# ArtoriasAbyssslayer/HashModNFFBanks-IDR

Hardware: AMD Instinct MI355X
Metric: rays/sec fwd+bwd (hash+SDF MLP) (higher is better)
Workload: dtype f32; 1 GPU; DTU-shaped synthetic uniform-sphere rays, MultiResHash L=16 T=2^19 F=2 (BASELINE.json configs[1]), full IDR training step (forward + IDRLoss + backward + clip + Adam), weights held at the geometric initialisation (lr = 0): the SURVEY.md 8(d) workload; grid_config=C2, rays_per_gpu=2048, global_rays=2048, parallelism=single GPU, world=1, ranks_seen=1, step=HIP-graph captured static-shape step

## Files before the change

hashmodnffbanks_idr_amd/csrc/hm_trace.hip:

```cpp
#include "hm_common.h"

#include <stdlib.h>
#include <string.h>

extern "C" int hm_trace_march_tail(const hm_grid_desc *desc, const hm_mlp_desc *mlp, const float *table,
                                   const float *B_fourier, int frac_mode, int body16, const void *trace_args, int first,
                                   int rounds, void *stream);

extern "C" int hm_trace_secant_persistent(const hm_grid_desc *desc, const hm_mlp_desc *mlp, const float *table,
                                          const float *B_fourier, int frac_mode, int tile_points, const void *trace_args,
                                          int n_iters, int scan_rule, void *stream);

extern "C" int hm_trace_scan_secant(const hm_grid_desc *desc, const hm_mlp_desc *mlp, const float *table,
                                    const float *B_fourier, int frac_mode, const void *trace_args, int n_iters,
                                    int64_t scan_off, int64_t scan_capacity, int c_prev1, int grid1, int c_prev2,
                                    int grid2, void *stream);

extern "C" int hm_sdf_fwd_fill(const hm_grid_desc *desc, const hm_mlp_desc *mlp, const float *x, int64_t n,
                               const float *table, const float *B_fourier, float *out, int frac_mode, const int32_t *n_dev,
                               const float *x_fill, float *out_fill, const int32_t *n_fill_dev, const int32_t *prev_dev,
                               int prev_grid, int *grid64_out, void *stream);

namespace {

constexpr int kTB = 256;

#include "hm_trace_dev.h"

__global__ __launch_bounds__(kTB) void trace_init_kernel(TraceArgs a) {
    const int64_t i = (int64_t)blockIdx.x * kTB + threadIdx.x;
    if (i >= a.n) return;
    trace_init_ray(a, i, a.w.cnt + C_ROUND0, 0);
}

__global__ __launch_bounds__(kTB) void trace_advance_kernel(TraceArgs a, int round) {
    const int64_t i = (int64_t)blockIdx.x * kTB + threadIdx.x;
    if (i >= a.n) return;
    trace_advance_ray(a, i, a.w.cnt + C_ROUND0 + round, 0);
}

__global__ __launch_bounds__(kTB) void trace_finalize_kernel(TraceArgs a) {
    const int64_t i = (int64_t)blockIdx.x * kTB + threadIdx.x;
    if (i >= a.n) return;
    const TraceWs &w = a.w;
    if (w.stage[i] != ST_DONE) atomicAdd(w.cnt + C_UNFINISHED, 1);
    const float t_s = w.t_s[i], t_e = w.t_e[i];
    a.out_mask[i] = t_s < t_e;
    a.out_t[i] = t_s;
    float px = 0.0f, py = 0.0f, pz = 0.0f;
    if (a.hit[i] || w.cnt[C_ANY_LIVE]) along(a, i, t_s, px, py, pz);
    a.out_pts[i * 3] = px; a.out_pts[i * 3 + 1] = py; a.out_pts[i * 3 + 2] = pz;
    const bool samp = w.live_s[i] != 0;
    w.is_samp[i] = samp;
    if (samp) w.list_samp[atomicAdd(w.cnt + C_NSAMP, 1)] = (int32_t)i;
}

__global__ __launch_bounds__(kTB) void ray_samples_kernel(TraceArgs a, const int32_t *list, int c_n, int c_npts,
                                                          const float *lo_arr, const float *hi_arr,
                                                          const float *fr, int c_base, int per_ray) {
    const int64_t gid = (int64_t)blockIdx.x * kTB + threadIdx.x;
    const TraceWs &w = a.w;
    const int32_t n_list = w.cnt[c_n];
    const int64_t base = c_base == -2 ? a.sel_off : (c_base >= 0 ? w.cnt[c_base] : 0);
    if (gid == 0) {
        w.cnt[c_npts] = n_list * per_ray;
        if (c_base != -2) w.cnt[C_BIG_PTS] = (int32_t)base + n_list * per_ray;
    }
    const int64_t m = gid / per_ray;
    if (m >= n_list) return;
    int s = (int)(gid - m * per_ray);
    if (per_ray < a.n_steps && s == per_ray - 1) s = a.n_steps - 1;
    const int64_t i = list[m];
    const float lo = lo_arr[i], hi = hi_arr[i];
    const float t = __fadd_rn(lo, __fmul_rn(fr[s], __fsub_rn(hi, lo)));
    float px, py, pz;
    along(a, i, t, px, py, pz);
    const int64_t o = base + gid;
    w.pts[o * 3] = px; w.pts[o * 3 + 1] = py; w.pts[o * 3 + 2] = pz;
}

__global__ __launch_bounds__(kTB) void sampler_head_kernel(TraceArgs a) {
    const int64_t m = (int64_t)blockIdx.x * kTB + threadIdx.x;
    const TraceWs &w = a.w;
    if (m >= w.cnt[C_NSAMP]) return;
    const int64_t i = w.list_samp[m];
    const float *v = w.vals + m * (a.head + 1);
    bool neg = false;
    for (int s = 0; s < a.head; ++s) neg = neg || (v[s] < 0.0f);
    const bool resolved = neg && a.obj[i] != 0;
    w.tail_slot[m] = resolved ? -1 : atomicAdd(w.cnt + C_NSAMP2, 1);
}

__global__ __launch_bounds__(kTB) void sampler_tail_points_kernel(TraceArgs a) {
    const int64_t gid = (int64_t)blockIdx.x * kTB + threadIdx.x;
    const TraceWs &w = a.w;
    const int per = a.n_steps - a.head - 1;
    if (gid == 0) {
        w.cnt[C_TAIL_PTS] = w.cnt[C_NSAMP2] * per;
        w.cnt[C_NSAMP_PTS] = w.cnt[C_HEAD_PTS] + w.cnt[C_NSAMP2] * per;
    }
    const int64_t m = gid / per;
    if (m >= w.cnt[C_NSAMP]) return;
    const int32_t q = w.tail_slot[m];
    if (q < 0) return;
    const int j = (int)(gid - m * per);
    const int64_t i = w.list_samp[m];
    const float lo = w.t_s[i], hi = w.t_e[i];
    const float t = __fadd_rn(lo, __fmul_rn(a.fracs[a.head + j], __fsub_rn(hi, lo)));
    float px, py, pz;
    along(a, i, t, px, py, pz);
    const int64_t o = a.tail_off + (int64_t)q * per + j;
    w.pts[o * 3] = px; w.pts[o * 3 + 1] = py; w.pts[o * 3 + 2] = pz;
}

__global__ __launch_bounds__(kTB) void sampler_reduce_kernel(TraceArgs a) {
    const int64_t m = (int64_t)blockIdx.x * kTB + threadIdx.x;
    const TraceWs &w = a.w;
    if (m >= w.cnt[C_NSAMP]) return;
    const int64_t i = w.list_samp[m];
    const int n = a.n_steps;
    const bool lazy = a.head > 0;
    const int32_t tq = lazy ? w.tail_slot[m] : 0;
    const float *v_head = lazy ? w.vals + m * (a.head + 1) : w.vals + m * n;
    const float *v_tail = lazy ? w.vals + a.tail_off + (int64_t)(tq < 0 ? 0 : tq) * (n - a.head - 1) - a.head : v_head;
    const int head = a.head;
    auto v = [&](int s) -> float {
        if (!lazy) return v_head[s];
        if (s < head) return v_head[s];
        return s == n - 1 ? v_head[head] : v_tail[s];
    };
    const int n_scan = (lazy && tq < 0) ? head : n;
    int first = 0, amin = 0, bad = 0;
    float best_tmp = 0.0f, best_v = 0.0f;
    auto visit = [&](int s, float x) {
        bad += !isfinite(x);
        const float sg = (x > 0.0f) ? 1.0f : ((x < 0.0f) ? -1.0f : 0.0f);
        const float tmp = sg * (float)(n - s);
        if (s == 0 || tmp < best_tmp) { best_tmp = tmp; first = s; }
        if (s == 0 || x < best_v) { best_v = x; amin = s; }
    };
    if (!lazy && (n & 3) == 0 && (reinterpret_cast<uintptr_t>(v_head) & 15u) == 0) {
        const float4 *row = reinterpret_cast<const float4 *>(v_head);
#pragma unroll 5
        for (int g4 = 0; g4 < n / 4; ++g4) {
            const float4 x4 = row[g4];
            visit(4 * g4, x4.x); visit(4 * g4 + 1, x4.y); visit(4 * g4 + 2, x4.z); visit(4 * g4 + 3, x4.w);
        }
    } else {
        for (int s = 0; s < n_scan; ++s) visit(s, v(s));
    }
    const float lo = w.t_s[i], hi = w.t_e[i];
    auto t_at = [&](int s) { return __fadd_rn(lo, __fmul_rn(a.fracs[s], __fsub_rn(hi, lo))); };
    const float v_first = v(first);
    const bool net_hit = v_first < 0.0f;
    const bool true_obj = a.obj[i] != 0;
    const int pick = (true_obj && net_hit) ? first : amin;
    float t_out = t_at(pick);
    float px, py, pz;
    along(a, i, t_out, px, py, pz);
    a.out_mask[i] = net_hit;
    const bool sec = a.training ? (net_hit && true_obj) : net_hit;
    if (sec) {
        const int lo_idx = first > 0 ? first - 1 : n - 1;
        const float z_hi = t_at(first), v_hi = v_first, z_lo = t_at(lo_idx), v_lo = v(lo_idx);
        if (lazy && tq < 0 && lo_idx == n - 1 && !isfinite(v_lo)) ++bad;
        const float z = secant_z(v_lo, v_hi, z_lo, z_hi);
        const int32_t q = atomicAdd(w.cnt + C_NSEC, 1);
        w.list_sec[q] = (int32_t)i;
        w.z_lo[q] = z_lo; w.z_hi[q] = z_hi; w.v_lo[q] = v_lo; w.v_hi[q] = v_hi; w.z[q] = z;
        if (a.n_secant == 0) {
            t_out = z;
            along(a, i, z, px, py, pz);
        }
    }
    if (bad) atomicAdd(w.cnt + C_NONFINITE, bad);
    a.out_t[i] = t_out;
    w.t_s[i] = t_out;
    a.out_pts[i * 3] = px; a.out_pts[i * 3 + 1] = py; a.out_pts[i * 3 + 2] = pz;
}

__global__ __launch_bounds__(kTB) void secant_points_kernel(TraceArgs a) {
    const int64_t q = (int64_t)blockIdx.x * kTB + threadIdx.x;
    const TraceWs &w = a.w;
    if (q >= w.cnt[C_NSEC]) return;
    float px, py, pz;
    along(a, w.list_sec[q], w.z[q], px, py, pz);
    w.pts[q * 3] = px; w.pts[q * 3 + 1] = py; w.pts[q * 3 + 2] = pz;
}

__global__ __launch_bounds__(kTB) void secant_advance_kernel(TraceArgs a, int last) {
    const int64_t q = (int64_t)blockIdx.x * kTB + threadIdx.x;
    if (q >= a.w.cnt[C_NSEC]) return;
    secant_advance_ray(a, q, last);
}

__global__ __launch_bounds__(kTB) void tail_prepare_kernel(TraceArgs a) {
    const int64_t i = (int64_t)blockIdx.x * kTB + threadIdx.x;
    if (i >= a.n) return;
    const TraceWs &w = a.w;
    const bool net = a.out_mask[i] != 0, obj = a.obj[i] != 0, samp = w.is_samp[i] != 0, hit = a.hit[i] != 0;
    const bool in_mask = !net && obj && !samp;
    const bool out_mask = !obj && !samp;
    if (!(in_mask || out_mask)) return;
    if (!hit) {
        const float *c = a.cam + (i / a.rays_per_image) * 3;
        const float *d = a.dirs + i * 3;
        const float dot = __fmaf_rn(d[2], c[2], __fmaf_rn(d[1], c[1], __fmul_rn(d[0], c[0])));
        const float t = -dot;
        float px, py, pz;
        along(a, i, t, px, py, pz);
        a.out_t[i] = t;
        w.t_s[i] = t;
        a.out_pts[i * 3] = px; a.out_pts[i * 3 + 1] = py; a.out_pts[i * 3 + 2] = pz;
        return;
    }
    if (net && out_mask) w.t_min[i] = w.t_s[i];
    w.list_sel[atomicAdd(w.cnt + C_NSEL, 1)] = (int32_t)i;
}

__global__ __launch_bounds__(kTB) void closest_reduce_kernel(TraceArgs a) {
    const int64_t m = (int64_t)blockIdx.x * kTB + threadIdx.x;
    const TraceWs &w = a.w;
    if (m >= w.cnt[C_NSEL]) return;
    const int64_t i = w.list_sel[m];
    const int n = a.n_steps;
    const float *v = w.vals + (a.sel_off >= 0 ? a.sel_off : (int64_t)w.cnt[a.head > 0 ? C_HEAD_PTS : C_NSAMP_PTS]) +
                     m * n;
    int amin = 0, bad = !isfinite(v[0]);
    float best = v[0];
    if ((n & 3) == 0 && (reinterpret_cast<uintptr_t>(v) & 15u) == 0) {
        const float4 *row = reinterpret_cast<const float4 *>(v);
        auto visit = [&](int s, float x) {
            if (s == 0) return;
            bad += !isfinite(x);
            if (x < best) { best = x; amin = s; }
        };
#pragma unroll 5
        for (int g4 = 0; g4 < n / 4; ++g4) {
            const float4 x4 = row[g4];
            visit(4 * g4, x4.x); visit(4 * g4 + 1, x4.y); visit(4 * g4 + 2, x4.z); visit(4 * g4 + 3, x4.w);
        }
    } else {
        for (int s = 1; s < n; ++s) {
            bad += !isfinite(v[s]);
            if (v[s] < best) { best = v[s]; amin = s; }
        }
    }
    if (bad) atomicAdd(w.cnt + C_NONFINITE, bad);
    const float lo = w.t_min[i], hi = w.t_max[i];
    const float t = __fadd_rn(__fmul_rn(a.steps_u[amin], __fsub_rn(hi, lo)), lo);
    float px, py, pz;
    along(a, i, t, px, py, pz);
    a.out_t[i] = t;
    a.out_pts[i * 3] = px; a.out_pts[i * 3 + 1] = py; a.out_pts[i * 3 + 2] = pz;
}

template <class V, class S, class O>
__device__ __forceinline__ void guard_mark_row(const TraceArgs &a, int n, bool signs, bool min_rule, bool true_obj,
                                               bool all, bool own_approx, bool other_approx, int c_ref, V val, S slot,
                                               O own) {
    const float tau = kGuardTau;
    const int kNone = 1 << 30;
    auto unc = [&](float x) { return !isfinite(x) || fabsf(x) <= tau; };
    int c = kNone;
    float m = INFINITY;
    for (int s = 0; s < n; ++s) {
        const float x = val(s);
        if (signs && c == kNone && x < -tau) c = s;
        if (isfinite(x) && x < m) m = x;
    }
    const bool use_min = min_rule && (!signs || !true_obj || c == kNone);
    const float lim = m + 2.0f * tau;
    auto marked = [&](int s, float x, float xn) -> bool {
        if (!(own(s) ? own_approx : other_approx)) return false;
        if (all && own(s)) return true;
        if (!isfinite(x)) return true;
        if (use_min && x <= lim) return true;
        if (!signs) return false;
        if (fabsf(x) <= tau || s == c) return true;
        const int nx = s + 1 == n ? 0 : s + 1;
        return nx <= c && (nx == c || unc(xn));
    };
    int n_mark = 0;
    float x = val(0);
    for (int s = 0; s < n; ++s) {
        const float xn = val(s + 1 == n ? 0 : s + 1);
        n_mark += marked(s, x, xn) ? 1 : 0;
        x = xn;
    }
    if (n_mark == 0) return;
    int64_t k = atomicAdd(a.w.cnt + c_ref, n_mark);
    x = val(0);
    for (int s = 0; s < n; ++s) {
        const float xn = val(s + 1 == n ? 0 : s + 1);
        if (marked(s, x, xn)) {
            const int64_t o = slot(s);
            a.w.ref_slot[k] = (int32_t)o;
            a.w.ref_pts[k * 3] = a.w.pts[o * 3]; a.w.ref_pts[k * 3 + 1] = a.w.pts[o * 3 + 1];
            a.w.ref_pts[k * 3 + 2] = a.w.pts[o * 3 + 2];
            ++k;
        }
        x = xn;
    }
}

__global__ __launch_bounds__(kTB) void guard_select_sampler_kernel(TraceArgs a, int pass, int c_live, int c_live2,
                                                                   int64_t min_live, int c_ref) {
    const int64_t m = (int64_t)blockIdx.x * kTB + threadIdx.x;
    const TraceWs &w = a.w;
    if (m >= w.cnt[C_NSAMP]) return;
    const bool approx = w.cnt[c_live] >= min_live, approx2 = c_live2 >= 0 && w.cnt[c_live2] >= min_live;
    if (!approx && !approx2) return;
    const bool all = *w.guard == kGuardTripped;
    const bool true_obj = a.obj[w.list_samp[m]] != 0;
    const int n = a.n_steps, head = a.head;
    if (pass == 1) {
        const int row = head > 0 ? head + 1 : n;
        const int64_t base = m * row;
        guard_mark_row(a, row, true, head == 0, true_obj, all, true, false, c_ref, [&](int s) { return w.vals[base + s]; },
                       [&](int s) { return base + s; }, [](int) { return true; });
        return;
    }
    const int32_t tq = w.tail_slot[m];
    if (tq < 0) return;
    const int64_t b_head = m * (head + 1), b_tail = a.tail_off + (int64_t)tq * (n - head - 1) - head;
    auto slot = [&](int s) -> int64_t { return s < head ? b_head + s : (s == n - 1 ? b_head + head : b_tail + s); };
    guard_mark_row(a, n, true, true, true_obj, all, approx, approx2, c_ref, [&](int s) { return w.vals[slot(s)]; }, slot,
                   [&](int s) { return s >= head && s != n - 1; });
}

__global__ __launch_bounds__(kTB) void guard_select_closest_kernel(TraceArgs a, int c_live, int64_t min_live, int c_ref) {
    const int64_t m = (int64_t)blockIdx.x * kTB + threadIdx.x;
    const TraceWs &w = a.w;
    if (m >= w.cnt[C_NSEL] || w.cnt[c_live] < min_live) return;
    const int n = a.n_steps;
    const int64_t base = (a.sel_off >= 0 ? a.sel_off : (int64_t)w.cnt[a.head > 0 ? C_HEAD_PTS : C_NSAMP_PTS]) + m * n;
    guard_mark_row(a, n, false, true, false, *w.guard == kGuardTripped, true, false, c_ref,
                   [&](int s) { return w.vals[base + s]; },
                   [&](int s) { return base + s; }, [](int) { return true; });
}

__global__ __launch_bounds__(kTB) void guard_patch_kernel(TraceArgs a, int c_ref) {
    const int64_t k = (int64_t)blockIdx.x * kTB + threadIdx.x;
    const TraceWs &w = a.w;
    const int32_t n_ref = w.cnt[c_ref];
    if (k == 0 && n_ref > 0) atomicAdd(w.cnt + C_GUARD_REFINED, n_ref);
    if (k >= n_ref) return;
    const int64_t o = w.ref_slot[k];
    const float e = w.ref_vals[k], ap = w.vals[o];
    if (isfinite(e) && isfinite(ap)) {
        const float d = fabsf(ap - e);
        if (d > 0.0f) atomicMax(w.cnt + C_GUARD_MAXDEV, __float_as_int(d));
        if (d > kGuardTrip) *w.guard = kGuardTripped;
    }
    w.vals[o] = e;
}

__global__ __launch_bounds__(kTB) void guard_noise_kernel(float *vals, int64_t off, const int32_t *n_live, int64_t min_live,
                                                          float amp, int nan_k) {
    const int64_t g = (int64_t)blockIdx.x * kTB + threadIdx.x;
    const int64_t n = *n_live;
    if (n < min_live || g >= n) return;
    const int64_t o = off + g;
    if (nan_k > 0) {
        if (o % nan_k == 0) vals[o] = ((o / nan_k) & 1) ? INFINITY : NAN;
        return;
    }
    uint32_t h = (uint32_t)o * 2654435761u;
    h ^= h >> 15; h *= 2246822519u; h ^= h >> 13;
    const float u = (float)(h >> 8) * (2.0f / 16777216.0f) - 1.0f;
    vals[o] = __fadd_rn(vals[o], __fmul_rn(amp, u));
}

__global__ void count_evals_kernel(int32_t *cnt, int rounds, int n_secant) {
    if (threadIdx.x != 0 || blockIdx.x != 0) return;
    int64_t tot = 0;
    for (int r = 0; r < rounds && r < 64; ++r) tot += cnt[C_ROUND0 + r];
    tot += cnt[C_NSAMP_PTS] + (int64_t)cnt[C_NSEC] * n_secant + cnt[C_NSEL_PTS];
    cnt[C_EVALS] = (int32_t)tot;
}

inline size_t align_up(size_t v, size_t a) { return (v + a - 1) / a * a; }

struct Layout {
    size_t off_f, off_i, off_b, off_pts, off_vals, off_cnt, off_emb, off_ref, total;
    int64_t cap;
};

constexpr size_t kWsHeader = 256;

Layout make_layout(int64_t n, int n_steps, int emb_width = 0, bool guard = false) {
    Layout L;
    L.cap = n * (n_steps > 2 ? n_steps : 2);
    size_t o = kWsHeader;
    L.off_f = o; o = align_up(o + sizeof(float) * 13 * (size_t)n, 256);
    L.off_i = o; o = align_up(o + sizeof(int32_t) * 6 * (size_t)n, 256);
    L.off_b = o; o = align_up(o + 6 * (size_t)n, 256);
    L.off_pts = o; o = align_up(o + sizeof(float) * 3 * 3 * (size_t)L.cap, 256);
    L.off_vals = o; o = align_up(o + sizeof(float) * 3 * (size_t)L.cap, 256);
    L.off_cnt = o; o = align_up(o + sizeof(int32_t) * C_COUNT, 256);
    L.off_emb = o; o = align_up(o + sizeof(float) * (size_t)emb_width * (size_t)L.cap, 256);
    L.off_ref = o; o = align_up(o + (guard ? sizeof(float) * 5 * (size_t)L.cap : 0), 256);
    L.total = o;
    return L;
}

}

extern "C" {

int64_t hm_trace_workspace_bytes(int64_t n_rays, const hm_trace_cfg *cfg) {
    if (n_rays < 0 || !cfg || cfg->n_steps < 1) return hm_fail(HM_ERR_INVALID, "hm_trace_workspace_bytes: bad argument");
    return (int64_t)make_layout(n_rays, cfg->n_steps, 0, cfg->coarse_bf16 == 3).total;
}

int hm_trace_guard_clear(void *workspace, int64_t workspace_bytes, void *stream) {
    HM_CHECK_ARG(workspace && workspace_bytes >= (int64_t)kWsHeader, "hm_trace_guard_clear: no workspace");
    hm_zero_u32_async(reinterpret_cast<int32_t *>(workspace), kWsHeader / sizeof(int32_t), as_stream(stream));
    HM_CHECK_LAUNCH("hm_trace_guard_clear");
    return HM_OK;
}

int hm_trace_guard_tolerances(float *tau, float *tau_trip) {
    HM_CHECK_ARG(tau && tau_trip, "hm_trace_guard_tolerances: NULL pointer");
    *tau = kGuardTau;
    *tau_trip = kGuardTrip;
    return HM_OK;
}

int64_t hm_trace_workspace_bytes_nffb(int64_t n_rays, const hm_trace_cfg *cfg, int n_levels) {
    if (n_rays < 0 || !cfg || cfg->n_steps < 1 || n_levels < 1 || n_levels > HM_MAX_LEVELS)
        return hm_fail(HM_ERR_INVALID, "hm_trace_workspace_bytes_nffb: bad argument");
    return (int64_t)make_layout(n_rays, cfg->n_steps, 3 + 8 + 8 * n_levels).total;
}

static int trace_forward_impl(const hm_grid_desc *desc, const hm_nffb_desc *nffb, const hm_mlp_desc *mlp,
                              const float *table, const float *B_fourier, int frac_mode, int tile_points,
                              const hm_trace_cfg *cfg, const float *cam_loc, const float *ray_dirs,
                              const uint8_t *object_mask, const float *t_sphere, const uint8_t *hit_mask, int64_t n_rays,
                              int64_t rays_per_image, const float *sampler_fracs, const float *steps_u,
                              float *out_points, uint8_t *out_net_mask, float *out_dists, void *workspace,
                              int64_t workspace_bytes, int32_t *stats_out, void *stream);

int hm_trace_forward(const hm_grid_desc *desc, const hm_mlp_desc *mlp, const float *table, const float *B_fourier,
                     int frac_mode, int tile_points, const hm_trace_cfg *cfg, const float *cam_loc,
                     const float *ray_dirs, const uint8_t *object_mask, const float *t_sphere,
                     const uint8_t *hit_mask, int64_t n_rays, int64_t rays_per_image, const float *sampler_fracs,
                     const float *steps_u, float *out_points, uint8_t *out_net_mask, float *out_dists,
                     void *workspace, int64_t workspace_bytes, int32_t *stats_out, void *stream) {
    return trace_forward_impl(desc, nullptr, mlp, table, B_fourier, frac_mode, tile_points, cfg, cam_loc, ray_dirs,
                              object_mask, t_sphere, hit_mask, n_rays, rays_per_image, sampler_fracs, steps_u, out_points,
                              out_net_mask, out_dists, workspace, workspace_bytes, stats_out, stream);
}

int hm_trace_forward_nffb(const hm_grid_desc *desc, const hm_nffb_desc *nffb, const hm_mlp_desc *mlp, const float *table,
                          const float *B_fourier, int frac_mode, int tile_points, const hm_trace_cfg *cfg,
                          const float *cam_loc, const float *ray_dirs, const uint8_t *object_mask, const float *t_sphere,
                          const uint8_t *hit_mask, int64_t n_rays, int64_t rays_per_image, const float *sampler_fracs,
                          const float *steps_u, float *out_points, uint8_t *out_net_mask, float *out_dists,
                          void *workspace, int64_t workspace_bytes, int32_t *stats_out, void *stream) {
    HM_CHECK_ARG(nffb != nullptr, "hm_trace_forward_nffb: NULL embedder descriptor");
    return trace_forward_impl(desc, nffb, mlp, table, B_fourier, frac_mode, tile_points, cfg, cam_loc, ray_dirs,
                              object_mask, t_sphere, hit_mask, n_rays, rays_per_image, sampler_fracs, steps_u, out_points,
                              out_net_mask, out_dists, workspace, workspace_bytes, stats_out, stream);
}

static int trace_forward_impl(const hm_grid_desc *desc, const hm_nffb_desc *nffb, const hm_mlp_desc *mlp,
                              const float *table, const float *B_fourier, int frac_mode, int tile_points,
                              const hm_trace_cfg *cfg, const float *cam_loc, const float *ray_dirs,
                              const uint8_t *object_mask, const float *t_sphere, const uint8_t *hit_mask, int64_t n_rays,
                              int64_t rays_per_image, const float *sampler_fracs, const float *steps_u,
                              float *out_points, uint8_t *out_net_mask, float *out_dists, void *workspace,
                              int64_t workspace_bytes, int32_t *stats_out, void *stream) {
    HM_CHECK_ARG(desc && mlp && cfg, "hm_trace_forward: NULL descriptor");
    HM_CHECK_ARG(n_rays >= 0 && rays_per_image >= 1, "hm_trace_forward: bad ray counts");
    HM_CHECK_ARG(cfg->n_steps >= 2 && cfg->n_steps <= 4096, "hm_trace_forward: n_steps out of range");
    HM_CHECK_ARG(cfg->sphere_tracing_iters >= 0 && cfg->sphere_tracing_iters <= 15 && cfg->line_step_iters >= 0 &&
                     cfg->line_step_iters <= 3 &&
                     1 + cfg->sphere_tracing_iters * (1 + cfg->line_step_iters) <= 64,
                 "hm_trace_forward: too many march rounds (sphere_tracing_iters <= 15, line_step_iters <= 3)");
    HM_CHECK_ARG(cfg->n_secant_steps >= 0 && cfg->n_secant_steps <= 64, "hm_trace_forward: n_secant_steps out of range");
    if (n_rays == 0) return HM_OK;
    HM_CHECK_ARG(n_rays * (int64_t)cfg->n_steps < (1ll << 31), "hm_trace_forward: too many rays for one call");
    HM_CHECK_ARG(table && B_fourier && cam_loc && ray_dirs && object_mask && t_sphere && hit_mask && sampler_fracs &&
                     out_points && out_net_mask && out_dists && workspace,
                 "hm_trace_forward: NULL pointer");
    HM_CHECK_ARG(!cfg->training || steps_u, "hm_trace_forward: training mode needs steps_u");
    HM_CHECK_ARG(cfg->coarse_bf16 >= 0 && cfg->coarse_bf16 <= 3, "hm_trace_forward: coarse_bf16 must be 0, 1, 2 or 3");
    const bool guard = cfg->coarse_bf16 == 3;
    HM_CHECK_ARG(!guard || !nffb, "hm_trace_forward: the guarded coarse scans do not cover filter-bank embedders");
    HM_CHECK_ARG(!guard || 3 * n_rays * (int64_t)cfg->n_steps < (1ll << 31), "hm_trace_forward: too many rays for one call");
    const int emb_width = nffb ? 3 + 8 + 8 * nffb->n_levels : 0;
    const Layout L = make_layout(n_rays, cfg->n_steps, emb_width, guard);
    HM_CHECK_ARG(workspace_bytes >= (int64_t)L.total, "hm_trace_forward: workspace too small");
    hipStream_t st = as_stream(stream);
    char *base = static_cast<char *>(workspace);
    const size_t n = (size_t)n_rays;
    TraceArgs a;
    float *f = reinterpret_cast<float *>(base + L.off_f);
    a.w.t_s = f; a.w.t_e = f + n; a.w.t_min = f + 2 * n; a.w.t_max = f + 3 * n; a.w.cur_s = f + 4 * n;
    a.w.cur_e = f + 5 * n; a.w.nxt_s = f + 6 * n; a.w.nxt_e = f + 7 * n; a.w.z_lo = f + 8 * n; a.w.z_hi = f + 9 * n;
    a.w.v_lo = f + 10 * n; a.w.v_hi = f + 11 * n; a.w.z = f + 12 * n;
    int32_t *ip = reinterpret_cast<int32_t *>(base + L.off_i);
    a.w.slot_s = ip; a.w.slot_e = ip + n; a.w.list_samp = ip + 2 * n; a.w.list_sec = ip + 3 * n; a.w.list_sel = ip + 4 * n;
    a.w.tail_slot = ip + 5 * n;
    uint8_t *bp = reinterpret_cast<uint8_t *>(base + L.off_b);
    a.w.live_s = bp; a.w.live_e = bp + n; a.w.stage = bp + 2 * n; a.w.it = bp + 3 * n; a.w.k = bp + 4 * n;
    a.w.is_samp = bp + 5 * n;
    a.w.pts = reinterpret_cast<float *>(base + L.off_pts);
    a.w.vals = reinterpret_cast<float *>(base + L.off_vals);
    a.w.cnt = reinterpret_cast<int32_t *>(base + L.off_cnt);
    a.w.cap = L.cap;
    a.w.ref_pts = reinterpret_cast<float *>(base + L.off_ref);
    a.w.ref_vals = a.w.ref_pts + 3 * (size_t)L.cap;
    a.w.ref_slot = reinterpret_cast<int32_t *>(a.w.ref_vals + (size_t)L.cap);
    a.w.guard = reinterpret_cast<int32_t *>(base);
    a.cam = cam_loc; a.dirs = ray_dirs; a.obj = object_mask; a.t_sphere = t_sphere; a.hit = hit_mask;
    a.fracs = sampler_fracs; a.steps_u = steps_u;
    a.out_pts = out_points; a.out_mask = out_net_mask; a.out_t = out_dists;
    a.n = n_rays; a.rays_per_image = rays_per_image;
    a.thr = cfg->sdf_threshold;
    for (int k = 0; k < 4; ++k) a.back[k] = (float)((1.0 - cfg->line_search_step) / (double)(1 << k));
    a.ls_iters = cfg->line_step_iters; a.max_it = cfg->sphere_tracing_iters; a.n_steps = cfg->n_steps;
    a.n_secant = cfg->n_secant_steps; a.training = cfg->training;
    a.head = (cfg->sampler_head >= 1 && cfg->sampler_head + 1 < cfg->n_steps) ? cfg->sampler_head : 0;
    a.tail_off = L.cap;
    const char *e_ov = getenv("HM_TRACE_OVERLAP");
    const bool overlap_ok = !(e_ov && atoi(e_ov) == 0);
    const bool overlap_shape = overlap_ok && cfg->training && !nffb && tile_points == 0 && cfg->n_secant_steps > 0 &&
                               n_rays <= kSdfSmall;
    const bool overlap = overlap_shape && !cfg->coarse_bf16;
    const bool sel_own = overlap || (guard && overlap_shape);
    a.sel_off = sel_own ? 2 * L.cap : -1;

    hm_zero_u32_async(a.w.cnt, C_COUNT, st);
    const unsigned g_rays = (unsigned)((n_rays + kTB - 1) / kTB);
    const unsigned g_samp = (unsigned)((n_rays * cfg->n_steps + kTB - 1) / kTB);

    float *emb_ws = reinterpret_cast<float *>(base + L.off_emb);
    auto sdf = [&](int64_t capacity, const int32_t *n_dev) -> int {
        if (nffb) {
            const int rc = hm_nffb_fwd(desc, nffb, a.w.pts, capacity, table, B_fourier, emb_ws, emb_width, frac_mode,
                                       n_dev, stream);
            if (rc != HM_OK) return rc;
            return hm_sdf_fwd_emb(mlp, emb_ws, emb_width, emb_width, capacity, a.w.vals, 1, 1, tile_points, n_dev, 0,
                                  stream);
        }
        return hm_sdf_fwd(desc, mlp, a.w.pts, capacity, table, B_fourier, a.w.vals, 1, 1, frac_mode, tile_points, n_dev,
                          0, stream);
    };
    auto coarse = [&](int64_t off, int64_t capacity, const int32_t *n_dev) -> int {
        const float *p = a.w.pts + off * 3;
        float *v = a.w.vals + off;
        const int64_t run_min = kSdfSmall + 1;
        int rc;
        if (!cfg->coarse_bf16) {
            if (nffb) {
                rc = hm_nffb_fwd(desc, nffb, p, capacity, table, B_fourier, emb_ws, emb_width, frac_mode, n_dev, stream);
                if (rc == HM_OK)
                    rc = hm_sdf_fwd_emb(mlp, emb_ws, emb_width, emb_width, capacity, v, 1, 1, tile_points, n_dev, 0, stream);
            } else {
                rc = hm_sdf_fwd(desc, mlp, p, capacity, table, B_fourier, v, 1, 1, frac_mode, tile_points, n_dev, 0, stream);
            }
        } else if (nffb) {
            rc = hm_nffb_fwd(desc, nffb, p, capacity, table, B_fourier, emb_ws, emb_width, frac_mode, n_dev, stream);
            if (rc == HM_OK)
                rc = hm_sdf_fwd_emb(mlp, emb_ws, emb_width, emb_width, capacity, v, 1, 1, -1, n_dev, 0, stream);
            if (rc == HM_OK)
                rc = cfg->coarse_bf16 == 2
                         ? hm_sdf_fwd_emb_split(mlp, emb_ws, emb_width, emb_width, capacity, v, 1, n_dev, run_min, stream)
                         : hm_sdf_fwd_emb_bf16(mlp, emb_ws, emb_width, emb_width, capacity, v, 1, n_dev, run_min, stream);
        } else if (guard && tile_points != 0) {
            rc = hm_sdf_fwd_split(desc, mlp, p, capacity, table, B_fourier, v, 1, frac_mode, n_dev, 1, stream);
        } else {
            rc = hm_sdf_fwd(desc, mlp, p, capacity, table, B_fourier, v, 1, 1, frac_mode, -1, n_dev, 0, stream);
            if (rc == HM_OK)
                rc = cfg->coarse_bf16 >= 2
                         ? hm_sdf_fwd_split(desc, mlp, p, capacity, table, B_fourier, v, 1, frac_mode, n_dev, run_min, stream)
                         : hm_sdf_fwd_bf16(desc, mlp, p, capacity, table, B_fourier, v, 1, frac_mode, n_dev, run_min, stream);
        }
        return rc;
    };
    const int64_t guard_min = tile_points == 0 ? kSdfSmall + 1 : 1;
    float noise_amp = 0.0f;
    int noise_nan = 0;
    if (guard) {
        const char *e = getenv("HM_TRACE_GUARD_NOISE");
        if (e && strncmp(e, "nan:", 4) == 0) noise_nan = atoi(e + 4) > 0 ? atoi(e + 4) : 0;
        else if (e) { const double f_ = atof(e); if (f_ > 0.0 && f_ < 1.0) noise_amp = (float)(f_ * kGuardTau); }
    }
    auto guard_noise = [&](int64_t off, int64_t capacity, int c_live) {
        if (noise_amp > 0.0f || noise_nan > 0)
            hipLaunchKernelGGL(guard_noise_kernel, dim3((unsigned)((capacity + kTB - 1) / kTB)), dim3(kTB), 0, st, a.w.vals,
                               off, a.w.cnt + c_live, guard_min, noise_amp, noise_nan);
    };
    auto guard_refine = [&](int c_ref) -> int {
        const int rc = hm_sdf_fwd(desc, mlp, a.w.ref_pts, L.cap, table, B_fourier, a.w.ref_vals, 1, 1, frac_mode,
                                  tile_points == 0 ? 64 : tile_points, a.w.cnt + c_ref, 0, stream);
        if (rc != HM_OK) return rc;
        hipLaunchKernelGGL(guard_patch_kernel, dim3((unsigned)((L.cap + kTB - 1) / kTB)), dim3(kTB), 0, st, a, c_ref);
        return HM_OK;
    };

    const int rounds = 1 + cfg->sphere_tracing_iters * (1 + cfg->line_step_iters);
    const bool tail = !nffb && (tile_points == 0 || tile_points == 16) &&
                      a.w.cap >= ((n_rays + 7) / 8) * 16 && cfg->line_step_iters > 0;
    int launched = tail ? 1 + cfg->sphere_tracing_iters : rounds;
    if (tail) {
        const char *e = getenv("HM_TRACE_TAIL_FIRST");
        const int k = e ? atoi(e) : 0;
        if (k >= 1 && k < launched) launched = k;
    }
    hipLaunchKernelGGL(trace_init_kernel, dim3(g_rays), dim3(kTB), 0, st, a);
    for (int r = 0; r < launched; ++r) {
        int rc = sdf(2 * n_rays, a.w.cnt + C_ROUND0 + r);
        if (rc != HM_OK) return rc;
        hipLaunchKernelGGL(trace_advance_kernel, dim3(g_rays), dim3(kTB), 0, st, a, r + 1 < 64 ? r + 1 : 63);
    }
    if (tail) {
        const int rc = hm_trace_march_tail(desc, mlp, table, B_fourier, frac_mode, tile_points == 16 ? 1 : 0, &a, launched,
                                           rounds, stream);
        if (rc != HM_OK) return rc;
    }
    hipLaunchKernelGGL(trace_finalize_kernel, dim3(g_rays), dim3(kTB), 0, st, a);

    if (cfg->training) hipLaunchKernelGGL(tail_prepare_kernel, dim3(g_rays), dim3(kTB), 0, st, a);
    const int per_ray = a.head > 0 ? a.head + 1 : cfg->n_steps;
    const int c_first = a.head > 0 ? (int)C_HEAD_PTS : (int)C_NSAMP_PTS;
    hipLaunchKernelGGL(ray_samples_kernel, dim3((unsigned)((n_rays * per_ray + kTB - 1) / kTB)), dim3(kTB), 0, st, a,
                       a.w.list_samp, (int)C_NSAMP, c_first, a.w.t_s, a.w.t_e, sampler_fracs, -1, per_ray);
    if (cfg->training)
        hipLaunchKernelGGL(ray_samples_kernel, dim3(g_samp), dim3(kTB), 0, st, a, a.w.list_sel, (int)C_NSEL,
                           (int)C_NSEL_PTS, a.w.t_min, a.w.t_max, steps_u, sel_own ? -2 : c_first, cfg->n_steps);
    int grid_p1 = 0, grid_p2 = 0;
    if (overlap) {
        int rc = hm_sdf_fwd_fill(desc, mlp, a.w.pts, n_rays * cfg->n_steps, table, B_fourier, a.w.vals, frac_mode,
                                 a.w.cnt + c_first, a.w.pts + a.sel_off * 3, a.w.vals + a.sel_off, a.w.cnt + C_NSEL_PTS,
                                 nullptr, 0, &grid_p1, stream);
        if (rc != HM_OK) return rc;
    } else {
        const int c_samp = sel_own ? c_first : (int)C_BIG_PTS, c_sel = sel_own ? (int)C_NSEL_PTS : (int)C_BIG_PTS;
        int rc = coarse(0, n_rays * cfg->n_steps, a.w.cnt + c_samp);
        if (rc == HM_OK && sel_own) rc = coarse(a.sel_off, n_rays * cfg->n_steps, a.w.cnt + c_sel);
        if (rc != HM_OK) return rc;
        if (guard) {
            guard_noise(0, n_rays * cfg->n_steps, c_samp);
            if (sel_own) guard_noise(a.sel_off, n_rays * cfg->n_steps, c_sel);
            hipLaunchKernelGGL(guard_select_sampler_kernel, dim3(g_rays), dim3(kTB), 0, st, a, 1, c_samp, -1, guard_min,
                               (int)C_GUARD_N1);
            if (cfg->training)
                hipLaunchKernelGGL(guard_select_closest_kernel, dim3(g_rays), dim3(kTB), 0, st, a, c_sel, guard_min,
                                   (int)C_GUARD_N1);
            rc = guard_refine((int)C_GUARD_N1);
            if (rc != HM_OK) return rc;
        }
    }
    if (cfg->training && !overlap) hipLaunchKernelGGL(closest_reduce_kernel, dim3(g_rays), dim3(kTB), 0, st, a);
    if (a.head > 0) {
        hipLaunchKernelGGL(sampler_head_kernel, dim3(g_rays), dim3(kTB), 0, st, a);
        hipLaunchKernelGGL(sampler_tail_points_kernel, dim3(g_samp), dim3(kTB), 0, st, a);
        int rc = overlap ? hm_sdf_fwd_fill(desc, mlp, a.w.pts + a.tail_off * 3, n_rays * (cfg->n_steps - a.head - 1), table,
                                           B_fourier, a.w.vals + a.tail_off, frac_mode, a.w.cnt + C_TAIL_PTS,
                                           a.w.pts + a.sel_off * 3, a.w.vals + a.sel_off, a.w.cnt + C_NSEL_PTS,
                                           a.w.cnt + c_first, grid_p1, &grid_p2, stream)
                         : coarse(a.tail_off, n_rays * (cfg->n_steps - a.head - 1), a.w.cnt + C_TAIL_PTS);
        if (rc != HM_OK) return rc;
        if (guard) {
            guard_noise(a.tail_off, n_rays * (cfg->n_steps - a.head - 1), (int)C_TAIL_PTS);
            hipLaunchKernelGGL(guard_select_sampler_kernel, dim3(g_rays), dim3(kTB), 0, st, a, 2, (int)C_TAIL_PTS,
                               sel_own ? c_first : (int)C_BIG_PTS, guard_min, (int)C_GUARD_N2);
            rc = guard_refine((int)C_GUARD_N2);
            if (rc != HM_OK) return rc;
        }
    }
    hipLaunchKernelGGL(sampler_reduce_kernel, dim3(g_rays), dim3(kTB), 0, st, a);
    if (cfg->n_secant_steps > 0) {
        hipLaunchKernelGGL(secant_points_kernel, dim3(g_rays), dim3(kTB), 0, st, a);
        if (overlap) {
            const int rc = hm_trace_scan_secant(desc, mlp, table, B_fourier, frac_mode, &a, cfg->n_secant_steps, a.sel_off,
                                                n_rays * cfg->n_steps, c_first, grid_p1, (int)C_TAIL_PTS, grid_p2, stream);
            if (rc != HM_OK) return rc;
            hipLaunchKernelGGL(closest_reduce_kernel, dim3(g_rays), dim3(kTB), 0, st, a);
        } else if (!nffb && (tile_points == 0 || tile_points == 4 || tile_points == 8 || tile_points == 16) &&
            (tile_points != 0 || n_rays <= kSdfSmall)) {
            const int rc = hm_trace_secant_persistent(desc, mlp, table, B_fourier, frac_mode, tile_points, &a,
                                                      cfg->n_secant_steps, sel_own ? 1 : 0, stream);
            if (rc != HM_OK) return rc;
        } else {
            for (int s = 0; s < cfg->n_secant_steps; ++s) {
                int rc = sdf(n_rays, a.w.cnt + C_NSEC);
                if (rc != HM_OK) return rc;
                hipLaunchKernelGGL(secant_advance_kernel, dim3(g_rays), dim3(kTB), 0, st, a,
                                   s == cfg->n_secant_steps - 1 ? 1 : 0);
            }
        }
    }
    hipLaunchKernelGGL(count_evals_kernel, dim3(1), dim3(64), 0, st, a.w.cnt, rounds + 1, cfg->n_secant_steps);
    if (stats_out) {
        hipLaunchKernelGGL(hm_copy_u32_kernel, dim3(1), dim3(64), 0, st, reinterpret_cast<uint32_t *>(stats_out),
                           reinterpret_cast<const uint32_t *>(a.w.cnt + C_NSAMP), 16);
    }
    HM_CHECK_LAUNCH("hm_trace_forward");
    return HM_OK;
}

}
```

Baseline: 274,400 rays/s.

## Parallelize guard row marking across a wavefront per ray

The guard selection kernels used one thread per ray, looping serially over all samples of the row. They now give each ray a 64-lane wavefront that strides over the samples. The min and first-negative-crossing values are combined with shuffle reductions, and ballot/popcount compacts the marked slots into the refine list under a single atomic per row. This cuts serial per-thread latency and gives coalesced reads, at the cost of launching 64x more threads. Only runs when the guard path is enabled.

```diff
diff --git a/hashmodnffbanks_idr_amd/csrc/hm_trace.hip b/hashmodnffbanks_idr_amd/csrc/hm_trace.hip
--- a/hashmodnffbanks_idr_amd/csrc/hm_trace.hip
+++ b/hashmodnffbanks_idr_amd/csrc/hm_trace.hip
@@ -255,19 +255,24 @@
     a.out_pts[i * 3] = px; a.out_pts[i * 3 + 1] = py; a.out_pts[i * 3 + 2] = pz;
 }
 
+constexpr int kGuardRows = kTB / 64;
 template <class V, class S, class O>
-__device__ __forceinline__ void guard_mark_row(const TraceArgs &a, int n, bool signs, bool min_rule, bool true_obj,
-                                               bool all, bool own_approx, bool other_approx, int c_ref, V val, S slot,
-                                               O own) {
+__device__ __forceinline__ void guard_mark_row(const TraceArgs &a, int lane, int n, bool signs, bool min_rule,
+                                               bool true_obj, bool all, bool own_approx, bool other_approx, int c_ref,
+                                               V val, S slot, O own) {
     const float tau = kGuardTau;
     const int kNone = 1 << 30;
     auto unc = [&](float x) { return !isfinite(x) || fabsf(x) <= tau; };
     int c = kNone;
     float m = INFINITY;
-    for (int s = 0; s < n; ++s) {
+    for (int s = lane; s < n; s += 64) {
         const float x = val(s);
         if (signs && c == kNone && x < -tau) c = s;
         if (isfinite(x) && x < m) m = x;
+    }
+    for (int d = 32; d > 0; d >>= 1) {
+        c = min(c, __shfl_xor(c, d));
+        m = fminf(m, __shfl_xor(m, d));
     }
     const bool use_min = min_rule && (!signs || !true_obj || c == kNone);
     const float lim = m + 2.0f * tau;
@@ -281,32 +286,32 @@
         const int nx = s + 1 == n ? 0 : s + 1;
         return nx <= c && (nx == c || unc(xn));
     };
+    auto mark_of = [&](int s) -> bool { return s < n && marked(s, val(s), val(s + 1 == n ? 0 : s + 1)); };
     int n_mark = 0;
-    float x = val(0);
-    for (int s = 0; s < n; ++s) {
-        const float xn = val(s + 1 == n ? 0 : s + 1);
-        n_mark += marked(s, x, xn) ? 1 : 0;
-        x = xn;
-    }
+    for (int s0 = 0; s0 < n; s0 += 64) n_mark += __popcll(__ballot(mark_of(s0 + lane)));
     if (n_mark == 0) return;
-    int64_t k = atomicAdd(a.w.cnt + c_ref, n_mark);
-    x = val(0);
-    for (int s = 0; s < n; ++s) {
-        const float xn = val(s + 1 == n ? 0 : s + 1);
-        if (marked(s, x, xn)) {
+    int k0 = 0;
+    if (lane == 0) k0 = atomicAdd(a.w.cnt + c_ref, n_mark);
+    int64_t k = __shfl(k0, 0);
+    for (int s0 = 0; s0 < n; s0 += 64) {
+        const int s = s0 + lane;
+        const bool mk = mark_of(s);
+        const unsigned long long b = __ballot(mk);
+        if (mk) {
+            const int64_t kk = k + __popcll(b & ((1ull << lane) - 1ull));
             const int64_t o = slot(s);
-            a.w.ref_slot[k] = (int32_t)o;
-            a.w.ref_pts[k * 3] = a.w.pts[o * 3]; a.w.ref_pts[k * 3 + 1] = a.w.pts[o * 3 + 1];
-            a.w.ref_pts[k * 3 + 2] = a.w.pts[o * 3 + 2];
-            ++k;
-        }
-        x = xn;
+            a.w.ref_slot[kk] = (int32_t)o;
+            a.w.ref_pts[kk * 3] = a.w.pts[o * 3]; a.w.ref_pts[kk * 3 + 1] = a.w.pts[o * 3 + 1];
+            a.w.ref_pts[kk * 3 + 2] = a.w.pts[o * 3 + 2];
+        }
+        k += __popcll(b);
     }
 }
 
 __global__ __launch_bounds__(kTB) void guard_select_sampler_kernel(TraceArgs a, int pass, int c_live, int c_live2,
                                                                    int64_t min_live, int c_ref) {
-    const int64_t m = (int64_t)blockIdx.x * kTB + threadIdx.x;
+    const int64_t m = (int64_t)blockIdx.x * kGuardRows + (threadIdx.x >> 6);
+    const int lane = threadIdx.x & 63;
     const TraceWs &w = a.w;
     if (m >= w.cnt[C_NSAMP]) return;
     const bool approx = w.cnt[c_live] >= min_live, approx2 = c_live2 >= 0 && w.cnt[c_live2] >= min_live;
@@ -317,25 +322,26 @@
     if (pass == 1) {
         const int row = head > 0 ? head + 1 : n;
         const int64_t base = m * row;
-        guard_mark_row(a, row, true, head == 0, true_obj, all, true, false, c_ref, [&](int s) { return w.vals[base + s]; },
-                       [&](int s) { return base + s; }, [](int) { return true; });
+        guard_mark_row(a, lane, row, true, head == 0, true_obj, all, true, false, c_ref,
+                       [&](int s) { return w.vals[base + s]; }, [&](int s) { return base + s; }, [](int) { return true; });
         return;
     }
     const int32_t tq = w.tail_slot[m];
     if (tq < 0) return;
     const int64_t b_head = m * (head + 1), b_tail = a.tail_off + (int64_t)tq * (n - head - 1) - head;
     auto slot = [&](int s) -> int64_t { return s < head ? b_head + s : (s == n - 1 ? b_head + head : b_tail + s); };
-    guard_mark_row(a, n, true, true, true_obj, all, approx, approx2, c_ref, [&](int s) { return w.vals[slot(s)]; }, slot,
-                   [&](int s) { return s >= head && s != n - 1; });
+    guard_mark_row(a, lane, n, true, true, true_obj, all, approx, approx2, c_ref, [&](int s) { return w.vals[slot(s)]; },
+                   slot, [&](int s) { return s >= head && s != n - 1; });
 }
 
 __global__ __launch_bounds__(kTB) void guard_select_closest_kernel(TraceArgs a, int c_live, int64_t min_live, int c_ref) {
-    const int64_t m = (int64_t)blockIdx.x * kTB + threadIdx.x;
+    const int64_t m = (int64_t)blockIdx.x * kGuardRows + (threadIdx.x >> 6);
+    const int lane = threadIdx.x & 63;
     const TraceWs &w = a.w;
     if (m >= w.cnt[C_NSEL] || w.cnt[c_live] < min_live) return;
     const int n = a.n_steps;
     const int64_t base = (a.sel_off >= 0 ? a.sel_off : (int64_t)w.cnt[a.head > 0 ? C_HEAD_PTS : C_NSAMP_PTS]) + m * n;
-    guard_mark_row(a, n, false, true, false, *w.guard == kGuardTripped, true, false, c_ref,
+    guard_mark_row(a, lane, n, false, true, false, *w.guard == kGuardTripped, true, false, c_ref,
                    [&](int s) { return w.vals[base + s]; },
                    [&](int s) { return base + s; }, [](int) { return true; });
 }
@@ -536,6 +542,7 @@
     hm_zero_u32_async(a.w.cnt, C_COUNT, st);
     const unsigned g_rays = (unsigned)((n_rays + kTB - 1) / kTB);
     const unsigned g_samp = (unsigned)((n_rays * cfg->n_steps + kTB - 1) / kTB);
+    const unsigned g_rows = (unsigned)((n_rays + kGuardRows - 1) / kGuardRows);
 
     float *emb_ws = reinterpret_cast<float *>(base + L.off_emb);
     auto sdf = [&](int64_t capacity, const int32_t *n_dev) -> int {
@@ -646,10 +653,10 @@
         if (guard) {
             guard_noise(0, n_rays * cfg->n_steps, c_samp);
             if (sel_own) guard_noise(a.sel_off, n_rays * cfg->n_steps, c_sel);
-            hipLaunchKernelGGL(guard_select_sampler_kernel, dim3(g_rays), dim3(kTB), 0, st, a, 1, c_samp, -1, guard_min,
+            hipLaunchKernelGGL(guard_select_sampler_kernel, dim3(g_rows), dim3(kTB), 0, st, a, 1, c_samp, -1, guard_min,
                                (int)C_GUARD_N1);
             if (cfg->training)
-                hipLaunchKernelGGL(guard_select_closest_kernel, dim3(g_rays), dim3(kTB), 0, st, a, c_sel, guard_min,
+                hipLaunchKernelGGL(guard_select_closest_kernel, dim3(g_rows), dim3(kTB), 0, st, a, c_sel, guard_min,
                                    (int)C_GUARD_N1);
             rc = guard_refine((int)C_GUARD_N1);
             if (rc != HM_OK) return rc;
@@ -667,7 +674,7 @@
         if (rc != HM_OK) return rc;
         if (guard) {
             guard_noise(a.tail_off, n_rays * (cfg->n_steps - a.head - 1), (int)C_TAIL_PTS);
-            hipLaunchKernelGGL(guard_select_sampler_kernel, dim3(g_rays), dim3(kTB), 0, st, a, 2, (int)C_TAIL_PTS,
+            hipLaunchKernelGGL(guard_select_sampler_kernel, dim3(g_rows), dim3(kTB), 0, st, a, 2, (int)C_TAIL_PTS,
                                sel_own ? c_first : (int)C_BIG_PTS, guard_min, (int)C_GUARD_N2);
             rc = guard_refine((int)C_GUARD_N2);
             if (rc != HM_OK) return rc;
```

Result: faster. 279,600 rays/s (median of 6 runs) (+1.9%).
